# y2w-oc/CMR-Agent

Measured on AMD Instinct MI355X. Metric: registration iters/sec (KITTI 352x1216 img + 16384 pts, 1 geo forward + 10 agent steps), higher is better.
Workload: dtype f32; 1 GPU; BASELINE.json configs[1]: KittiConfig, batch 8 per GPU, 16384 pts, 352x1216 image, 10 agent steps, fp32, hash-filled weights; batch_per_gpu=8, parallelism=batch sharding, no data-path collective

## Files before the change

cmr_agent_amd/models/MultiHeadModel.py:

```python
import itertools
import math

import numpy as np
import torch
import torch.nn as nn

from .. import ops
from ..utils.streams import fork_join
from . import _pack
from ._pack import Planned
from .ImageResNet import ResidualBlock
from .IMGPCEnDecoder import IMGPCEnDecoder
from .PointNN import ConvBNReLURes1D, bcl_from_rows

HEAD_SLOPE = 0.2


class _Head(Planned):

    def __init__(self, config, pc_out, img_out, pc_name, img_name, pc_mid, img_mid):
        super().__init__()
        self.config = config
        f = config.embed_dim
        self.point_fuse_convs = nn.ModuleList([ConvBNReLURes1D(2 * f, f)] +
                                              [ConvBNReLURes1D(f, f) for _ in range(config.pt_head_res_num - 1)])
        setattr(self, pc_name, nn.Sequential(nn.Conv1d(f, pc_mid, kernel_size=1, stride=1, padding=0),
                                             nn.LeakyReLU(HEAD_SLOPE, inplace=True),
                                             nn.Conv1d(pc_mid, pc_out, kernel_size=1, stride=1, padding=0)))
        self.img_res_convs = nn.ModuleList([ResidualBlock(f, f) for _ in range(config.img_fuse_res_num)])
        setattr(self, img_name, nn.Sequential(nn.Conv2d(f, img_mid, 1, 1, 0), nn.LeakyReLU(HEAD_SLOPE, inplace=True),
                                              nn.Conv2d(img_mid, img_out, 1, 1, 0)))
        self._pc_name, self._img_name = pc_name, img_name
        self._pc_out, self._img_out = pc_out, img_out

    def _build_plan(self):
        pc, im = getattr(self, self._pc_name), getattr(self, self._img_name)
        return dict(pc0=_pack.lin(pc[0]), pc2=_pack.lin(pc[2]), im0=_pack.lin(im[0]), im2=_pack.lin(im[2]))

    def points_cl(self, cl):
        self._require_eval()
        p = self.plan()
        x = self.point_fuse_convs[0].rows(cl["pt_feat"], x2=cl["fused_node_feat"], idx2=cl["geo"].gidx)
        for layer in list(self.point_fuse_convs)[1:]:
            x = layer.rows(x)
        pts = ops.linear(ops.linear(x, *p["pc0"], act=ops.ACT_LRELU, act_param=HEAD_SLOPE), *p["pc2"])
        return pts[:, :self._pc_out]

    def pixels_cl(self, cl):
        self._require_eval()
        p = self.plan()
        y = cl["fused_img_feat"]
        for layer in self.img_res_convs:
            y = layer.forward_cl(y)
        B, h, w, f = y.shape
        pix = ops.linear(ops.linear(y.view(B * h * w, f), *p["im0"], act=ops.ACT_LRELU, act_param=HEAD_SLOPE), *p["im2"])
        return pix[:, :self._img_out]

    def trunk_cl(self, cl):
        return fork_join(lambda: self.points_cl(cl), lambda: self.pixels_cl(cl), tag="trunk")


class OverlapDetectionHead(_Head):
    def __init__(self, config):
        super().__init__(config, 2, 2, "pc_overlap_head", "img_overlap_head", 32, 32)

    def finish_cl(self, cl, pts, pix):
        cl["pc_overlap_logits"], cl["img_overlap_logits"] = pts, pix
        return cl

    def forward_cl(self, cl):
        return self.finish_cl(cl, *self.trunk_cl(cl))


MATCH_INLIER_THRES = 3.0
SUBPIXEL_INLIER_THRES = 0.5


def point_xy_float_all(K, pc_in_cam_space):
    K = K.float()
    pc_ = torch.matmul(K if K.dim() == 3 else K.unsqueeze(0), pc_in_cam_space.float())
    return (pc_[:, 0:2, :] / pc_[:, 2:3, :]).contiguous()


def _gt_xy(data_batch, dev):
    xy = data_batch.get('point_xy_float_all')
    if xy is None:
        xy = point_xy_float_all(data_batch['K'].to(dev), data_batch['pc_in_cam_space'].to(dev))
    return xy.to(dev, torch.float32).contiguous()


def _geo_rows(data_batch):
    cl = data_batch.get('_cmr')
    if cl is not None and 'pc_geo_feat' in cl and 'img_geo_feat' in cl:
        return cl['pc_geo_feat'].contiguous(), cl['img_geo_feat'].contiguous()
    pcb, imb = data_batch['pc_geo_feat'], data_batch['img_geo_feat']
    return pcb.permute(0, 2, 1).reshape(-1, pcb.shape[1]).contiguous(), imb.permute(0, 2, 3, 1).contiguous()


def match_features(data_batch, mask, img_overlap=None, want_dist=False):
    pc, img = _geo_rows(data_batch)
    B, h, w, _ = img.shape
    N = pc.shape[0] // B
    dev = pc.device
    xy = _gt_xy(data_batch, dev)
    idx, dist, counts = ops.feat_match(pc, img, mask.to(dev).contiguous(), gt_xy=xy, thr=MATCH_INLIER_THRES, img_overlap=img_overlap,
                                       want_dist=want_dist)
    return idx.view(B, N), dist, counts, w


def match_features_filtered(data_batch, mask, mutual=True, ratio=0.0, excl_radius=2, max_dist=0.0):
    pc, img = _geo_rows(data_batch)
    B, h, w, _ = img.shape
    N = pc.shape[0] // B
    dev = pc.device
    idx, keep, counts, _, _, _ = ops.feat_match_filter(pc, img, mask.to(dev).contiguous(), mutual=mutual, ratio=ratio,
                                                       excl_radius=excl_radius, max_dist=max_dist, gt_xy=_gt_xy(data_batch, dev),
                                                       thr=MATCH_INLIER_THRES)
    return idx.view(B, N), keep.view(B, N), counts, w


def match_features_conf(data_batch, mask, temperature=0.1, min_conf=0.0):
    pc, img = _geo_rows(data_batch)
    B, h, w, _ = img.shape
    N = pc.shape[0] // B
    dev = pc.device
    idx, conf, keep, counts, _, _, _ = ops.match_conf(pc, img, mask.to(dev).contiguous(), temperature=temperature, min_conf=min_conf,
                                                      gt_xy=_gt_xy(data_batch, dev), thr=MATCH_INLIER_THRES)
    return idx.view(B, N), conf.view(B, N), keep.view(B, N), counts, w


def _ratio(counts, num, den):
    c = counts.float()
    return c[:, num] / c[:, den]


class GeometricDistanceHead(_Head):
    def __init__(self, config):
        f = config.embed_dim
        super().__init__(config, f, f, "pc_geo_head", "img_geo_head", f, f)
        self.dist_thres, self.pos_margin, self.neg_margin, self.lambda_geo = 1, 0.1, 1.4, 1

    def finish_cl(self, cl, pts, pix):
        cl["pc_geo_feat"] = ops.l2norm64(pts)
        cl["img_geo_feat"] = ops.l2norm64(pix).view(cl["B"], cl["h"], cl["w"], -1)
        return cl

    def forward_cl(self, cl):
        return self.finish_cl(cl, *self.trunk_cl(cl))

    def cal_match_accuracy(self, data_batch):
        with torch.no_grad():
            _, _, counts, _ = match_features(data_batch, data_batch['pc_mask'])
            ir = _ratio(counts, 1, 0)
            data_batch['matching_ir_per_sample'] = ir
            data_batch['matching_ir'] = ir[0]


_EYE4 = {}


def _eye4(dev):
    key = str(dev)
    if key not in _EYE4:
        _EYE4[key] = torch.eye(4, device=dev).unsqueeze(0)
    return _EYE4[key]


SEARCH_LEVELS = ((4, 1.0, 0.1, 3), (2, 0.5, 0.05, 3), (1, 0.25, 0.025, 3), (0, 0.1, 0.01, 6), (0, 0.03, 0.003, 6))


def pose_search_offsets():
    return np.array(sorted(itertools.product((-1, 0, 1), repeat=6), key=lambda o: (sum(abs(x) for x in o), o)), np.int64)


def pose_search_table(rot_step_deg, trans_step):
    o = pose_search_offsets().astype(np.float64)
    wv = math.radians(float(rot_step_deg)) * o[:, :3]
    th = np.linalg.norm(wv, axis=1)
    W = np.zeros((len(o), 3, 3))
    W[:, 0, 1], W[:, 0, 2], W[:, 1, 2] = -wv[:, 2], wv[:, 1], -wv[:, 0]
    W[:, 1, 0], W[:, 2, 0], W[:, 2, 1] = wv[:, 2], -wv[:, 1], wv[:, 0]
    small = th < 1e-8
    ths = np.where(small, 1.0, th)
    a = np.where(small, 1.0 - th * th / 6.0, np.sin(ths) / ths)
    c = np.where(small, 0.5 - th * th / 24.0, (1.0 - np.cos(ths)) / (ths * ths))
    D = np.tile(np.eye(4), (len(o), 1, 1))
    D[:, :3, :3] += a[:, None, None] * W + c[:, None, None] * (W @ W)
    D[:, :3, 3] = float(trans_step) * o[:, 3:]
    return torch.from_numpy(D)


def _first_min(score):
    P = score.shape[1]
    ar = torch.arange(P, device=score.device)
    k = torch.where(score == score.min(1, keepdim=True).values, ar, torch.full_like(ar, P)).min(1).values
    return torch.where(k < P, k, torch.zeros_like(k))

# ... 434 lines not shown
```

cmr_agent_amd/models/PointNN.py:

```python
import torch
import torch.nn as nn

from .. import ops
from . import _pack
from ._pack import Planned


def rows_from_bcl(x, cpad=None):
    B, C, L = x.shape
    xp = x.permute(0, 2, 1)
    if cpad is None and xp.is_contiguous():
        return xp.reshape(B * L, C)
    if cpad is not None:
        return ops.planar_to_rows(x.contiguous(), cpad)
    return ops.transpose(x.contiguous()).view(B * L, C)


def bcl_from_rows(r, B):
    return r.view(B, -1, r.shape[1]).permute(0, 2, 1)


class MiniPointNet(Planned):
    SLOPE = 0.2

    def __init__(self, in_channels=3, out_channels=64):
        super().__init__()
        self.in_channels = in_channels
        mk = lambda ci: nn.Sequential(nn.Conv1d(ci, out_channels, kernel_size=1, stride=1, padding=0),
                                      nn.BatchNorm1d(out_channels), nn.LeakyReLU(self.SLOPE, inplace=True))
        self.layer_1, self.layer_2, self.layer_3 = mk(in_channels), mk(out_channels), mk(out_channels)

    def _build_plan(self):
        return [_pack.lin(l[0], l[1]) for l in (self.layer_1, self.layer_2, self.layer_3)]

    def rows(self, x1, x2=None, idx2=None, div2=1):
        self._require_eval()
        p = self.plan()
        y = ops.linear(x1, *p[0], x2=x2, idx2=idx2, div2=div2, act=ops.ACT_LRELU, act_param=self.SLOPE)
        y = ops.linear(y, *p[1], act=ops.ACT_LRELU, act_param=self.SLOPE)
        return ops.linear(y, *p[2], act=ops.ACT_LRELU, act_param=self.SLOPE)

    def forward(self, x):
        B = x.shape[0]
        r = rows_from_bcl(x, 4 if self.in_channels < 4 else None)
        return bcl_from_rows(self.rows(r), B)


class ConvBNReLURes1D(Planned):
    SLOPE = 0.2

    def __init__(self, in_channels=3, out_channels=3):
        super().__init__()
        self.in_channels, self.out_channels = in_channels, out_channels
        self.net = nn.Sequential(nn.Conv1d(in_channels, in_channels, kernel_size=1, stride=1, padding=0),
                                 nn.BatchNorm1d(in_channels), nn.LeakyReLU(self.SLOPE, inplace=True),
                                 nn.Conv1d(in_channels, out_channels, kernel_size=1, stride=1, padding=0),
                                 nn.BatchNorm1d(out_channels))
        self.final_relu = nn.LeakyReLU(self.SLOPE, inplace=True)
        if in_channels == out_channels:
            self.shortcut = nn.Identity()
        else:
            self.shortcut = nn.Sequential(nn.Conv1d(in_channels, out_channels, kernel_size=1, stride=1, padding=0),
                                          nn.BatchNorm1d(out_channels))

    def _build_plan(self):
        w1, b1 = _pack.lin(self.net[0], self.net[1])
        w1, b1 = _pack.pad_rows(w1, b1)
        w2, b2 = _pack.lin(self.net[3], self.net[4])
        sc = None if isinstance(self.shortcut, nn.Identity) else _pack.lin(self.shortcut[0], self.shortcut[1])
        b2f = b2 if sc is None else (b2 + sc[1]).contiguous()
        return dict(l1=(w1, b1), l2=(w2, b2), sc=sc, b2f=b2f)

    def rows(self, x1, x2=None, idx2=None, div2=1, res_rows=None):
        self._require_eval()
        p = self.plan()
        fused = ops.cbr_block(x1, p["l1"][0], p["l1"][1], p["l2"][0], p["b2f"], None if p["sc"] is None else p["sc"][0],
                              self.SLOPE, x2=x2, idx2=idx2, div2=div2)
        if fused is not None:
            return fused[0]
        hid = ops.linear(x1, *p["l1"], x2=x2, idx2=idx2, div2=div2, act=ops.ACT_LRELU, act_param=self.SLOPE)
        if p["sc"] is not None:
            res = ops.linear(x1, *p["sc"], x2=x2, idx2=idx2, div2=div2)
        elif x2 is None:
            res = x1
        else:
            res = res_rows if res_rows is not None else ops.concat_rows(x1, x2, idx2, div2)
        return ops.linear(hid, *p["l2"], res=res, act=ops.ACT_LRELU, act_param=self.SLOPE)

    def forward(self, x):
        B = x.shape[0]
        r = rows_from_bcl(x, 8 if self.in_channels == 5 else (4 if self.in_channels < 4 else None))
        return bcl_from_rows(self.rows(r), B)


FUSED_FRONT = True


def _vector_attention(p, q, k, v, rel, rows, nseg, iq, divq, ik, order, offsets, fixed_len):
    pos = ops.linear(ops.linear(rel, *p["d0"], act=ops.ACT_RELU), *p["d2"])
    t, vp = ops.vecattn_prep(q, k, v, pos, rows, iq=iq, divq=divq, ik=ik)
    a = ops.linear(ops.linear(t, *p["g0"], act=ops.ACT_RELU), *p["g2"])
    return ops.segment_softmax(a, vp, nseg, 0.125, order=order, offsets=offsets, fixed_len=fixed_len)


class GroupPointTransformer(Planned):
    def __init__(self, d_points=3, d_model=128):
        super().__init__()
        if d_model != 64:
            raise NotImplementedError("vector-attention kernels are instantiated for d_model = 64")
        c1 = lambda ci, co, bias=True: nn.Conv1d(ci, co, kernel_size=1, stride=1, padding=0, bias=bias)
        self.fc1_0, self.fc1_1, self.fc2 = c1(d_points, d_model), c1(d_points, d_model), c1(d_model, d_points)
        self.fc_delta = nn.Sequential(c1(3, d_model), nn.ReLU(inplace=True), c1(d_model, d_model))
        self.fc_gamma = nn.Sequential(c1(d_model, d_model), nn.ReLU(inplace=True), c1(d_model, d_model))
        self.w_qs, self.w_ks, self.w_vs = c1(d_model, d_model, False), c1(d_model, d_model, False), c1(d_model, d_model, False)
        self.d_model = d_model

    def _build_plan(self):
        wk, _ = _pack.lin(self.w_ks)
        wv, _ = _pack.lin(self.w_vs)
        return dict(fc1_0=_pack.lin(self.fc1_0), fc1_1=_pack.lin(self.fc1_1), fc2=_pack.lin(self.fc2),
                    d0=_pack.lin(self.fc_delta[0]), d2=_pack.lin(self.fc_delta[2]), g0=_pack.lin(self.fc_gamma[0]),
                    g2=_pack.lin(self.fc_gamma[2]), wq=_pack.lin(self.w_qs)[0], wkv=torch.cat([wk, wv], 0).contiguous())

    def rows(self, xyz4, feat, node4, node_feat, gidx, offsets, order):
        self._require_eval()
        p = self.plan()
        R, S = feat.shape[0], node_feat.shape[0]
        q = ops.linear(ops.linear(node_feat, *p["fc1_1"]), p["wq"])
        if FUSED_FRONT and p["d0"][0].shape == (64, 4):
            a, vp = ops.vecattn_front(q, xyz4, node4, gidx, p["d0"], p["d2"], p["g0"], p["g2"], R, iq=gidx, feat=feat,
                                      fc1=p["fc1_0"], wkv=p["wkv"])
            res = ops.segment_softmax(a, vp, S, 0.125, order=order, offsets=offsets, fixed_len=0)
        else:
            kv = ops.linear(ops.linear(feat, *p["fc1_0"]), p["wkv"])
            rel = ops.rel_pos(xyz4, node4, R, ib=gidx)
            res = _vector_attention(p, q, kv[:, 0:64], kv[:, 64:128], rel, R, S, gidx, 1, None, order, offsets, 0)
        return ops.linear(res, *p["fc2"], res=node_feat)

    def forward(self, xyz, xyz_features, node, node_features, idx):
        B, N, M = xyz.shape[0], xyz.shape[2], node.shape[2]
        gidx = ops.index_to_global(idx.contiguous(), M)
        offsets, order = ops.csr_build(gidx, B, N, M)
        out = self.rows(rows_from_bcl(xyz, 4), rows_from_bcl(xyz_features), rows_from_bcl(node, 4),
                        rows_from_bcl(node_features), gidx, offsets, order)
        return bcl_from_rows(out, B)


class KnnPointTransformer(Planned):
    def __init__(self, d_points=3, d_model=128, k=16):
        super().__init__()
        if d_model != 64 or k != 16:
            raise NotImplementedError("kNN transformer kernels are instantiated for d_model = 64, k = 16")
        self.fc1, self.fc2 = nn.Linear(d_points, d_model), nn.Linear(d_model, d_points)
        self.fc_delta = nn.Sequential(nn.Linear(3, d_model), nn.ReLU(inplace=True), nn.Linear(d_model, d_model))
        self.fc_gamma = nn.Sequential(nn.Linear(d_model, d_model), nn.ReLU(inplace=True), nn.Linear(d_model, d_model))
        self.w_qs = nn.Linear(d_model, d_model, bias=False)
        self.w_ks = nn.Linear(d_model, d_model, bias=False)
        self.w_vs = nn.Linear(d_model, d_model, bias=False)
        self.k = k

    def _build_plan(self):
        wq, wk, wv = (_pack.lin(l)[0] for l in (self.w_qs, self.w_ks, self.w_vs))
        return dict(fc1=_pack.lin(self.fc1), fc2=_pack.lin(self.fc2), d0=_pack.lin(self.fc_delta[0]),
                    d2=_pack.lin(self.fc_delta[2]), g0=_pack.lin(self.fc_gamma[0]), g2=_pack.lin(self.fc_gamma[2]),
                    wqkv=torch.cat([wq, wk, wv], 0).contiguous())

    def rows(self, node4, feat, knn):
        self._require_eval()
        p = self.plan()
        S = feat.shape[0]
        qkv = ops.linear(ops.linear(feat, *p["fc1"]), p["wqkv"])
        if FUSED_FRONT and p["d0"][0].shape == (64, 4):
            a, vp = ops.vecattn_front(qkv[:, 0:64], node4, node4, knn, p["d0"], p["d2"], p["g0"], p["g2"], S * 16, divq=16,
                                      diva=16, kv=qkv[:, 64:192], ik=knn)
            res = ops.segment_softmax(a, vp, S, 0.125, fixed_len=16)
        else:
            rel = ops.rel_pos(node4, node4, S * 16, diva=16, ib=knn)
            res = _vector_attention(p, qkv[:, 0:64], qkv[:, 64:128], qkv[:, 128:192], rel, S * 16, S, None, 16, knn, None,
                                    None, 16)
        return ops.linear(res, *p["fc2"], res=feat)

    def forward(self, xyz, features):
        B, M = xyz.shape[0], xyz.shape[2]
        node4 = rows_from_bcl(xyz, 4)
        knn = ops.knn16(node4, B, M).view(-1)
        return bcl_from_rows(self.rows(node4, rows_from_bcl(features), knn), B)
```

cmr_agent_amd/ops.py:

```python
import math
import os

import torch

from . import _lib

ACT_NONE, ACT_RELU, ACT_LRELU, ACT_GELU, ACT_ELU1 = 0, 1, 2, 3, 4
f32 = torch.float32
GRID_Y_MAX = 65535


def _stream():
    return torch.cuda.current_stream().cuda_stream


def _p(t):
    return None if t is None else t.data_ptr()


def _rows(t, name="tensor"):
    if t.dim() != 2 or t.stride(1) != 1 or t.dtype != f32 or not t.is_cuda:
        raise ValueError("%s must be a 2-D float32 device tensor with unit inner stride, got %s %s %s" % (
            name, tuple(t.shape), t.stride(), t.dtype))
    return t
# ... 44 lines not shown
        k2 = x2.shape[1]
    if kw != k1 + k2 or w.stride(1) != 1 or w.stride(0) < kw:
        raise ValueError("weight shape %s / strides %s do not match k1+k2=%d" % (tuple(w.shape), w.stride(), k1 + k2))
    ldw = w.stride(0) if n_out > 1 else kw
    if out is None:
        out = torch.empty((rows, n_out), dtype=f32, device=x1.device)
    _rows(out, "out")
    if res is not None:
        _rows(res, "res")
    if _AB_SKIP_LINEAR:
        key = (rows, n_out, x1.device)
        if key not in _AB_ZERO:
            _AB_ZERO[key] = torch.zeros((rows, n_out), dtype=f32, device=x1.device)
        return _AB_ZERO[key]
    if CONV_BF16 and LINEAR_BF16 and x2 is None and ldw == kw and rows >= LINEAR_BF16_MIN_ROWS and k1 in (32, 64, 128) and n_out <= 128 and n_out % 4 == 0:
        rc = _lib.call("cmr_linear_rows_bf16_f32", _p(x1), _ld(x1), k1, _p(w), kw, _p(bias), _p(res), _ld(res) if res is not None else 0,
                       int(res_mod), _p(out), _ld(out), rows, n_out, act, float(act_param), _stream(), allow_unsupported=True)
        if rc != _lib.UNSUPPORTED:
            return out
    _lib.call("cmr_linear_f32", _p(x1), _ld(x1), k1, _p(x2), _ld(x2) if x2 is not None else 0, k2, _p(_i32(idx2)),
              int(div2), _p(w), ldw, _p(bias), _p(res), _ld(res) if res is not None else 0, int(res_mod), _p(out),
              _ld(out), rows, n_out, act, float(act_param), _stream())
    return out


def cbr_block(x1, w1, b1, w2, b2, wsc, slope, x2=None, idx2=None, div2=1, rows_per_batch=None, want_y=True,
              want_colmax=False):
    _rows(x1, "x1")
    rows, k1 = x1.shape
    kx = k1 + (x2.shape[1] if x2 is not None else 0)
    ch, co = w1.shape[0], w2.shape[0]
    if w1.shape[1] != kx or w2.shape[1] != ch or (wsc is not None and tuple(wsc.shape) != (co, kx)):
        raise ValueError("cbr_block: inconsistent weight shapes")
    rpb = rows if rows_per_batch is None else rows_per_batch
    B = rows // rpb
    if want_colmax and (rpb % 32 or rows % rpb):
        return None
    y = torch.empty((rows, co), dtype=f32, device=x1.device) if want_y else None
    ntiles = (rows + 31) // 32
    part = torch.empty((ntiles, co), dtype=f32, device=x1.device) if want_colmax else None
    s1 = b1.stride(0) if b1.dim() == 2 else 0
    s2 = b2.stride(0) if b2.dim() == 2 else 0
    rc = _lib.call("cmr_cbr_block_bf16_f32" if CONV_BF16 else "cmr_cbr_block_f32", _p(x1), _ld(x1), k1, _p(x2), _ld(x2) if x2 is not None else 0, _p(_i32(idx2)),
                   int(div2), kx, ch, co, _p(w1), _p(b1), s1, _p(w2), _p(b2), s2, _p(wsc), _p(y), co, _p(part), rows, rpb,
                   float(slope), _stream(), allow_unsupported=True)
    if rc == _lib.UNSUPPORTED:
        return None
    cm = None
    if want_colmax == "partials":
        return y, part
    if want_colmax:
        cm = colmax_partials(part, B, rpb // 32)
    return y, cm


def colmax_partials(part, B, tiles_per_batch):
    co = part.shape[1]
    cm = torch.empty((B, co), dtype=f32, device=part.device)
    _lib.call("cmr_colmax_partials_f32", _p(part), _p(cm), B, int(tiles_per_batch), co, _stream())
    return cm


COLMAX_BIAS2 = os.environ.get("CMR_COLMAX_BIAS2", "fp32")


def colmax_bias2(part, B, tiles_per_batch, w1, b1, w2, b2, want_g=False):
    C = part.shape[1]
    n1, n2 = w1.shape[0], w2.shape[0]
    if COLMAX_BIAS2 == "0" or (COLMAX_BIAS2 == "fp32" and CONV_BF16) or C != 64 or n1 % 4 or n2 % 4 or not (w1.is_contiguous() and w2.is_contiguous()) or w1.shape[1] != C or w2.shape[1] != C:
        return None
    y1 = torch.empty((B, n1), dtype=f32, device=part.device)
    y2 = torch.empty((B, n2), dtype=f32, device=part.device)
    g = torch.empty((B, C), dtype=f32, device=part.device) if want_g else None
    rc = _lib.call("cmr_colmax_bias2_f32", _p(part), B, int(tiles_per_batch), C, _p(w1), _p(b1), n1, _p(w2), _p(b2), n2, _p(g), _p(y1), _p(y2), _stream(),
                   allow_unsupported=True)
    return None if rc == _lib.UNSUPPORTED else (y1, y2, g)


def layernorm64(x, gamma, beta, eps, res=None, out=None):
    _rows(x, "x")
    if out is None:
        out = torch.empty((x.shape[0], 64), dtype=f32, device=x.device)
    _lib.call("cmr_layernorm64_f32", _p(x), _ld(x), _p(gamma), _p(beta), float(eps), _p(res),
              _ld(res) if res is not None else 0, _p(out), _ld(out), x.shape[0], _stream())
    return out


CONV_BF16 = False
BF16_CHAINS = True
BF16_STORE = True
STRIDE2_FRAGS = True
WINOGRAD = True
WINO_MIN_TILES = 64


TOWER_CU_BUDGET = 160
TOWER_CU_BUDGET_F32 = 0


TOWER_SLICES_F32 = int(os.environ.get("CMR_TOWER_SLICES", "1"))


import threading

_policy = threading.local()

# ... 2035 lines not shown
```

cmr_agent_amd/utils/workmodel.py:

```python
import torch

from .. import _lib

FP32_MFMA_PEAK = 157.3e12
HBM_PEAK = 8.0e12
RIDGE = FP32_MFMA_PEAK / HBM_PEAK
F = 4


def _linear(a):
    rows, k1, n = a["rows"], a["k1"], a["n_out"]
    k2 = a["k2"] if a["x2"] else 0
    src2 = 0
    if a["x2"]:
        src2 = rows * k2 if a["idx2"] else max(rows // max(a["div2"], 1), 1) * k2
    by = F * (rows * k1 + src2 + rows * n + n * (k1 + k2) + (rows * n if a["res"] and not a["res_mod"] else 0))
    return 2.0 * rows * (k1 + k2) * n, by


def _cbr(a):
    rows, kx, ch, co, k1 = a["rows"], a["kx"], a["ch"], a["co"], a["k1"]
    w = kx * ch + ch * co + (kx * co if a["wsc"] else 0)
    src2 = 0
    if a["x2"]:
        src2 = rows * (kx - k1) if a["idx2"] else max(rows // max(a["div2"], 1), 1) * (kx - k1)
    return 2.0 * rows * w, F * (rows * k1 + src2 + (rows * co if a["y"] else 0) + w)


def _conv(a, stride=None):
    s = a.get("stride", 1) if stride is None else stride
    B, H, W, ci, co, pool = a["B"], a["H"], a["W"], a["Cin"], a["Cout"], a.get("pool", 1)
    opix = B * ((H - 1) // s + 1) * ((W - 1) // s + 1)
    by = F * (B * H * W * ci + opix * co / (pool * pool) + (opix * co if a["res"] else 0) + 9 * ci * co)
    return 2.0 * 9 * ci * co * opix, by


def _conv_io(a):
    s = a.get("stride", 1)
    B, H, W, ci, co, pool = a["B"], a["H"], a["W"], a["Cin"], a["Cout"], a.get("pool", 1)
    opix = B * ((H - 1) // s + 1) * ((W - 1) // s + 1)
    by = ((2 if a["x_bf16"] else F) * B * H * W * ci + (2 if a["y_bf16"] else F) * opix * co / (pool * pool)
          + (2 if a.get("res_bf16") else F) * (opix * co if a["res"] else 0) + F * 9 * ci * co)
    return 2.0 * 9 * ci * co * opix, by


def _heads(a):
    w = 2 * 128 * 128 + sum(256 * a[p + "_n0"] + a[p + "_n0"] * a[p + "_n1"] + a[p + "_n1"] * a[p + "_n2"] for p in "rtv")
    return 2.0 * a["B"] * w, F * (a["B"] * a["npix"] * 128 + w)


def _vecattn(a):
    rows = a["rows"]
    if a["feat"]:
        return rows * 2.0 * (3 * 4096 + 192 + 4096 + 2 * 4096), rows * (256 + 256 + 32 + 512)
    return rows * 2.0 * (192 + 4096 + 2 * 4096), rows * (512 + 256 + 32 + 512)


WORK = {
    "cmr_linear_f32": _linear,
    "cmr_cbr_block_f32": _cbr,
    "cmr_cbr_block_bf16_f32": _cbr,
    "cmr_colmax_partials_f32": lambda a: (0, F * a["B"] * a["tiles_per_batch"] * a["C"]),
    "cmr_colmax_bias2_f32": lambda a: (2.0 * a["B"] * a["C"] * (a["n1"] + a["n2"]),
                                       F * (a["B"] * a["tiles_per_batch"] * a["C"] + (a["C"] + 1 + a["B"]) * (a["n1"] + a["n2"]))),
    "cmr_layernorm64_f32": lambda a: (0, F * a["rows"] * 64 * (3 if a["res"] else 2)),
    "cmr_conv3x3_nhwc_f32": _conv,
    "cmr_conv3x3_wino_nhwc_f32": lambda a: _conv(a, 1),
    "cmr_conv3x3_wino_stats_nhwc_f32": lambda a: (2.0 * 9 * a["Cin"] * a["Cout"] * a["B"] * a["H"] * a["W"],
                                                  F * (a["B"] * a["H"] * a["W"] * (a["Cin"] + a["Cout"]) + 9 * a["Cin"] * a["Cout"])),
    "cmr_bn_stats_from_sums_f32": lambda a: (0, F * a["parts"] * 2 * a["C"]),
    "cmr_conv3x3_wino_bnbwd_nhwc_f32": lambda a: (2.0 * 9 * a["Cin"] * a["Cout"] * a["B"] * a["H"] * a["W"],
                                                  F * (a["B"] * a["H"] * a["W"] * (a["Cin"] + 2 * a["Cout"]) + 9 * a["Cin"] * a["Cout"])),
    "cmr_bn_bwd_from_sums_f32": lambda a: (0, F * a["rows"] * a["C"] * 3),
    "cmr_conv3x3_s2_nhwc_f32": lambda a: _conv(a, 2),
    "cmr_conv3x3_bf16_nhwc_f32": _conv,
    "cmr_conv3x3_bf16io_nhwc": _conv_io,
    "cmr_conv3x3_bf16_pro_nhwc_f32": lambda a: (2.0 * 9 * a["Cin"] * a["Cout"] * a["B"] * a["H"] * a["W"],
                                                F * (a["B"] * a["H"] * a["W"] * (a["Cin"] + a["Cout"]) + 9 * a["Cin"] * a["Cout"])),
    "cmr_stem_block_f32": lambda a: (2.0 * (81 + 1728 + 192) * a["B"] * a["H"] * a["W"], a["B"] * a["H"] * a["W"] * (F * 3 + (2 if a.get("out_bf16") else F) * 64)),
    "cmr_avgpool_nhwc_f32": lambda a: (0, F * a["B"] * a["H"] * a["W"] * a["C"] * (1 + 1.0 / (a["kh"] * a["kw"]))),
    "cmr_upsample_concat_f32": lambda a: (0, F * a["B"] * a["H"] * a["W"] * (2 * a["C1"] + a["C2"] * (1 + 1.0 / a["scale"] ** 2))),
    "cmr_patchify_nhwc_f32": lambda a: (0, 2 * F * a["B"] * a["H"] * a["W"] * a["C"]),
    "cmr_transpose_f32": lambda a: (0, 2 * F * a["batch"] * a["R"] * a["Cn"]),
    "cmr_linear_rows_bf16_f32": lambda a: (2.0 * a["rows"] * a["k"] * a["n_out"], F * (a["rows"] * (a["k"] + a["n_out"] * (2 if a["res"] else 1)) + a["k"] * a["n_out"])),
    "cmr_patch_embed_f32": lambda a: (2.0 * a["B"] * (a["H"] // a["P"]) * (a["W"] // a["P"]) * a["P"] * a["P"] * a["C"] * a["n_out"],
                                     F * (a["B"] * a["H"] * a["W"] * a["C"] + a["B"] * (a["H"] // a["P"]) * (a["W"] // a["P"]) * a["n_out"] + a["P"] * a["P"] * a["C"] * a["n_out"])),
    "cmr_mha_f32": lambda a: (4.0 * a["B"] * a["Tq"] * a["Tk"] * 64, F * 64 * a["B"] * (2 * a["Tq"] + 2 * a["Tk"])),
    "cmr_mha_expf_f32": lambda a: (4.0 * a["B"] * a["Tq"] * a["Tk"] * 64, F * 64 * a["B"] * (2 * a["Tq"] + 2 * a["Tk"])),
    "cmr_mha_ln_f32": lambda a: (4.0 * a["B"] * a["Tq"] * a["Tk"] * 64 + 2.0 * 64 * a["B"] * (64 * a["Tq"] + 128 * a["Tk"]),
                                F * 64 * a["B"] * (2 * a["Tq"] + a["Tk"])),
    "cmr_la_reduce_f32": lambda a: (2.0 * a["B"] * a["S"] * 576, F * a["B"] * a["S"] * 128),
    "cmr_la_apply_f32": lambda a: (2.0 * a["B"] * a["L"] * 576, F * a["B"] * a["L"] * 128),
    "cmr_agent_heads_f32": _heads,
    "cmr_agent_heads_train_f32": _heads,
    "cmr_ln64_linear_f32": lambda a: (2.0 * 64 * (a["rows_x"] * a["n_out_x"] + (a["rows_y"] * a["n_out_y"] if a["y"] else 0)),
                                      F * (a["rows_x"] * (64 + a["n_out_x"]) + (a["rows_y"] * (64 + a["n_out_y"]) if a["y"] else 0)
                                           + 64 * (a["n_out_x"] + (a["n_out_y"] if a["y"] else 0)))),
    "cmr_ln64_linear_bf16_f32": lambda a: (2.0 * 64 * (a["rows_x"] * a["n_out_x"] + (a["rows_y"] * a["n_out_y"] if a["y"] else 0)),
                                      F * (a["rows_x"] * (64 + a["n_out_x"]) + (a["rows_y"] * (64 + a["n_out_y"]) if a["y"] else 0)
                                           + 64 * (a["n_out_x"] + (a["n_out_y"] if a["y"] else 0)))),
    "cmr_vit_out_ffn_f32": lambda a: (2.0 * a["rows"] * (4096 + 2 * 65536), F * (a["rows"] * 192 + 4096 + 2 * 65536)),
    "cmr_vit_out_ffn16_f32": lambda a: (2.0 * a["rows"] * (4096 + 2 * 65536), F * (a["rows"] * 192 + 4096 + 2 * 65536)),
    "cmr_vit_out_ffn_bf16_f32": lambda a: (2.0 * a["rows"] * (4096 + 2 * 65536), F * (a["rows"] * 192 + 4096 + 2 * 65536)),
    "cmr_la_kv_state_f32": lambda a: (2.0 * a["B"] * a["S"] * (2 * 4096 + 576), F * (a["B"] * a["S"] * 64 + 2 * 4096)),
    "cmr_la_kv_state_bf16_f32": lambda a: (2.0 * a["B"] * a["S"] * (2 * 4096 + 576), F * (a["B"] * a["S"] * 64 + 2 * 4096)),
    "cmr_la_query_layer_f32": lambda a: (2.0 * a["B"] * a["L"] * (4096 + 576 + 4096 + 16384 + 8192),
                                         F * (a["B"] * a["L"] * 128 + 2 * 4096 + 16384 + 8192)),
    "cmr_la_query_layer_bf16_f32": lambda a: (2.0 * a["B"] * a["L"] * (4096 + 576 + 4096 + 16384 + 8192),
                                         F * (a["B"] * a["L"] * 128 + 2 * 4096 + 16384 + 8192)),
    "cmr_vecattn_front_f32": _vecattn,
    "cmr_focal_metrics_f32": lambda a: (0, a["rows"] * 16),
    "cmr_circle_loss_f32": lambda a: (2.0 * a["B"] * a["n"] * a["n"] * 64, F * a["B"] * a["n"] * 128),
    "cmr_planar_to_rows_f32": lambda a: (0, F * a["B"] * a["N"] * (a["C"] + a["Cpad"])),
# ... 189 lines not shown
```

include/cmr_hip.h:

```cpp
#ifndef CMR_HIP_H
#define CMR_HIP_H
#include <stdint.h>

#ifdef __cplusplus
extern "C" {
#endif

typedef struct ihipStream_t* hipStream_t;

#define CMR_OK 0
#define CMR_EINVAL -1
#define CMR_ELAUNCH -2
#define CMR_EUNSUPPORTED -3

enum { CMR_ACT_NONE = 0, CMR_ACT_RELU = 1, CMR_ACT_LRELU = 2, CMR_ACT_GELU = 3, CMR_ACT_ELU1 = 4 };


int cmr_linear_f32(const float* x1, int64_t ld1, int k1, const float* x2, int64_t ld2, int k2, const int32_t* idx2,
                   int64_t div2, const float* w, int64_t ldw, const float* bias, const float* res, int64_t ldres,
                   int64_t res_mod, float* y, int64_t ldy, int64_t rows, int n_out, int act, float act_param,
                   hipStream_t stream);
int cmr_cbr_block_f32(const float* x1, int64_t ld1, int k1, const float* x2, int64_t ld2, const int32_t* idx2,
                      int64_t div2, int kx, int ch, int co, const float* w1, const float* b1, int64_t b1_stride,
                      const float* w2, const float* b2, int64_t b2_stride, const float* wsc, float* y, int64_t ldy,
                      float* colmax_part, int64_t rows, int64_t rows_per_batch, float slope, hipStream_t stream);
int cmr_cbr_block_bf16_f32(const float* x1, int64_t ld1, int k1, const float* x2, int64_t ld2, const int32_t* idx2,
                           int64_t div2, int kx, int ch, int co, const float* w1, const float* b1, int64_t b1_stride,
                           const float* w2, const float* b2, int64_t b2_stride, const float* wsc, float* y, int64_t ldy,
                           float* colmax_part, int64_t rows, int64_t rows_per_batch, float slope, hipStream_t stream);
int cmr_colmax_partials_f32(const float* part, float* out, int B, int tiles_per_batch, int C, hipStream_t stream);
int cmr_colmax_bias2_f32(const float* part, int B, int tiles_per_batch, int C, const float* w1, const float* b1, int n1, const float* w2,
                         const float* b2, int n2, float* g, float* y1, float* y2, hipStream_t stream);

int cmr_layernorm64_f32(const float* x, int64_t ldx, const float* gamma, const float* beta, float eps, const float* res,
                        int64_t ldres, float* y, int64_t ldy, int64_t rows, hipStream_t stream);

int cmr_conv3x3_nhwc_f32(const float* x, int B, int H, int W, int Cin, const float* w, const float* bias,
                         const float* res, const float* post, float* y, int Cout, int stride, float slope, int pool,
                         hipStream_t stream);

int cmr_conv3x3_wino_nhwc_f32(const float* x, int B, int H, int W, int Cin, const float* u, const float* bias,
                              const float* res, const float* post, float* y, int Cout, float slope, int pool,
                              int cu_budget, int slices, hipStream_t stream);
int64_t cmr_conv3x3_wino_stats_parts(int B, int H, int W, int Cin, int Cout, int cu_budget, int slices);
int cmr_conv3x3_wino_stats_nhwc_f32(const float* x, int B, int H, int W, int Cin, const float* u, const float* bias, float* y, int Cout,
                                    int cu_budget, int slices, float* part, int64_t parts, hipStream_t stream);
int cmr_conv3x3_wino_bnbwd_nhwc_f32(const float* dy, int B, int H, int W, int Cin, const float* u, float* dx, int Cout, const float* bn_x,
                                    const float* bn_stat, float bn_slope, int cu_budget, int slices, float* part, int64_t parts,
                                    hipStream_t stream);
int cmr_conv3x3_s2_nhwc_f32(const float* x, int B, int H, int W, int Cin, const float* wfrag, const float* bias, const float* res,
                            const float* post, float* y, int Cout, float slope, hipStream_t stream);
int cmr_stem_block_f32(const float* x_nchw, const float* w_a, const float* b_a, const float* w3, const float* w1,
                       const float* b_b, float* tmp_nchw, void* y_nhwc, int out_bf16, int B, int H, int W, float slope,
                       hipStream_t stream);

int cmr_avgpool_nhwc_f32(const float* x, float* y, int B, int H, int W, int C, int kh, int kw, hipStream_t stream);

int cmr_upsample_concat_f32(const float* f, const float* proxy, float* out, int B, int H, int W, int C1, int C2,
                            int scale, hipStream_t stream);

int cmr_patchify_nhwc_f32(const float* x, float* out, int B, int H, int W, int C, int P, hipStream_t stream);
int cmr_patch_embed_f32(const float* x_nhwc, int B, int H, int W, int C, int P, const float* w, int64_t ldw, const float* bias,
                        const float* res, int64_t ldres, int64_t res_mod, float* y, int64_t ldy, int n_out, hipStream_t stream);
int cmr_linear_rows_bf16_f32(const float* x, int64_t ldx, int k, const float* w, int64_t ldw, const float* bias, const float* res,
                             int64_t ldres, int64_t res_mod, float* y, int64_t ldy, int64_t rows, int n_out, int act, float act_param,
                             hipStream_t stream);

int cmr_transpose_f32(const float* x, float* y, int batch, int R, int Cn, hipStream_t stream);


int cmr_mha_f32(const float* q, int64_t ldq, const float* k, int64_t ldk, const float* v, int64_t ldv, float* o,
                int64_t ldo, int B, int Tq, int Tk, hipStream_t stream);
int cmr_mha_expf_f32(const float* q, int64_t ldq, const float* k, int64_t ldk, const float* v, int64_t ldv, float* o, int64_t ldo, int B,
                     int Tq, int Tk, hipStream_t stream);
int cmr_mha_ln_f32(const float* x, int64_t ldx, const float* y, int64_t ldy, const float* gamma, const float* beta, float eps,
                   const float* wq_frag, const float* wkv_frag, const float* bq, const float* bk, const float* bv, float* o, int64_t ldo,
                   int B, int Tq, int Tk, hipStream_t stream);
int64_t cmr_la_reduce_workspace_bytes(int B, int S);
int cmr_la_reduce_f32(const float* kf, int64_t ldk, const float* v, int64_t ldv, float* kvsum, void* workspace,
                      int64_t workspace_bytes, int B, int S, hipStream_t stream);
int cmr_la_apply_f32(const float* qf, int64_t ldq, const float* kvsum, float* msg, int64_t ldm, int B, int L, int S,
                     float eps, hipStream_t stream);

// ... 449 lines not shown
```

Baseline: 418.4 registration iters/s.

## Fuse chains of row-wise linear layers into one LDS-resident MFMA kernel

```diff
diff --git a/cmr_agent_amd/csrc/row_chain.hip b/cmr_agent_amd/csrc/row_chain.hip
--- /dev/null
+++ b/cmr_agent_amd/csrc/row_chain.hip
@@ -0,0 +1,244 @@
+#include "cmr_common.h"
+
+namespace {
+
+__device__ __attribute__((aligned(16))) float rc_zero[16] = {0.f};
+
+struct RcArgs {
+  const float* x1; int64_t ld1;
+  const float* x2; int64_t ld2; const int32_t* idx2; int64_t div2;
+  int k1;
+  const float* w1; const float* b1;
+  const float* w2; const float* b2;
+  const float* w3; const float* b3;
+  float s1, s2, s3;
+  float* y; int64_t ldy;
+  int64_t rows;
+};
+
+template <int C, int K, int KP>
+__device__ __forceinline__ void rc_stage(float* Ws, float* Bs, const float* __restrict__ w, const float* __restrict__ b, int tid) {
+  constexpr int P = 32 * ((C + 31) / 32), LD = KP + 4;
+  for (int e = tid; e < P * (KP / 4); e += 512) {
+    const int n = e / (KP / 4), c = (e % (KP / 4)) * 4;
+    const bool ok = n < C && c < K;
+    *reinterpret_cast<f32x4*>(&Ws[n * LD + c]) = *reinterpret_cast<const f32x4*>(ok ? w + (int64_t)n * K + c : rc_zero);
+  }
+  for (int e = tid; e < P; e += 512) Bs[e] = (b && e < C) ? b[e] : 0.f;
+}
+
+template <int G, int T, int LD>
+__device__ __forceinline__ void rc_gemm(const float* wl, const f32x4 (&in)[G], f32x16 (&acc)[T]) {
+#pragma unroll
+  for (int t = 0; t < T; ++t)
+#pragma unroll
+    for (int r = 0; r < 16; ++r) acc[t][r] = 0.f;
+  f32x4 wc[T], wn[T];
+#pragma unroll
+  for (int t = 0; t < T; ++t) wc[t] = *reinterpret_cast<const f32x4*>(wl + t * 32 * LD);
+#pragma unroll
+  for (int g = 0; g < G; ++g) {
+    if (g + 1 < G) {
+#pragma unroll
+      for (int t = 0; t < T; ++t) wn[t] = *reinterpret_cast<const f32x4*>(wl + t * 32 * LD + (g + 1) * 8);
+    }
+#pragma unroll
+    for (int j = 0; j < 4; ++j)
+#pragma unroll
+      for (int t = 0; t < T; ++t) acc[t] = cmr_mfma32(wc[t][j], in[g][j], acc[t]);
+    __builtin_amdgcn_sched_barrier(0);
+#pragma unroll
+    for (int t = 0; t < T; ++t) wc[t] = wn[t];
+  }
+}
+
+template <int T>
+__device__ __forceinline__ void rc_act(const f32x16 (&acc)[T], const float* bl, float slope, f32x4 (&out)[4 * T]) {
+#pragma unroll
+  for (int t = 0; t < T; ++t)
+#pragma unroll
+    for (int q = 0; q < 4; ++q) {
+      const f32x4 bv = *reinterpret_cast<const f32x4*>(bl + t * 32 + q * 8);
+#pragma unroll
+      for (int e = 0; e < 4; ++e) {
+        const float v = acc[t][4 * q + e] + bv[e];
+        out[4 * t + q][e] = v > 0.f ? v : v * slope;
+      }
+    }
+}
+
+template <int G, int TL, int TC, int LD, int CL, bool NORM>
+__device__ __forceinline__ void rc_last(const float* wl, const float* bl, const f32x4 (&in)[G], float slope, float* yrow, bool valid, int h) {
+  static_assert(!NORM || (CL == 64 && TL == 2 && TC == 2), "l2norm epilogue: 64 channels");
+#pragma unroll
+  for (int c0 = 0; c0 < TL; c0 += TC) {
+    f32x16 acc[TC];
+    rc_gemm<G, TC, LD>(wl + c0 * 32 * LD, in, acc);
+    f32x4 ov[4 * TC];
+    rc_act<TC>(acc, bl + c0 * 32, slope, ov);
+    if constexpr (NORM) {
+      float s[8];
+#pragma unroll
+      for (int i = 0; i < 8; ++i) {
+        const float p = fmaf(ov[i][0], ov[i][0], ov[i][1] * ov[i][1]) + fmaf(ov[i][2], ov[i][2], ov[i][3] * ov[i][3]);
+        s[i] = p + cmr_xhalf(p);
+      }
+      const float qq = ((s[0] + s[1]) + (s[2] + s[3])) + ((s[4] + s[5]) + (s[6] + s[7]));
+      const float d = fmaxf(sqrtf(qq), 1e-12f);
+#pragma unroll
+      for (int i = 0; i < 8; ++i)
+#pragma unroll
+        for (int e = 0; e < 4; ++e) ov[i][e] = ov[i][e] / d;
+    }
+#pragma unroll
+    for (int i = 0; i < 4 * TC; ++i) cmr_pin(ov[i]);
+    if (valid) {
+#pragma unroll
+      for (int t = 0; t < TC; ++t)
+#pragma unroll
+        for (int q = 0; q < 4; ++q) {
+          const int c = (c0 + t) * 32 + q * 8;
+          if (c + 8 <= CL) *reinterpret_cast<f32x4*>(yrow + c) = ov[4 * t + q];
+          else if (c + 4 <= CL && h == 0) *reinterpret_cast<f32x4*>(yrow + c) = ov[4 * t + q];
+        }
+    }
+  }
+}
+
+template <int K0, int C1, int C2, int C3, bool NORM>
+__global__ __launch_bounds__(512) void row_chain_kernel(const RcArgs a) {
+  constexpr int KP = K0 < 8 ? 8 : K0, GX = KP / 8;
+  constexpr bool THREE = C3 > 0;
+  constexpr int T1 = (C1 + 31) / 32, T2 = (C2 + 31) / 32, T3 = (C3 + 31) / 32;
+  constexpr int LD1 = KP + 4, LD2 = C1 + 4, LD3 = C2 + 4;
+  constexpr int CL = THREE ? C3 : C2, TL = THREE ? T3 : T2, TC = TL >= 2 ? 2 : 1;
+  static_assert(C1 % 32 == 0 && (!THREE || C2 % 32 == 0) && CL % 4 == 0 && TL % TC == 0 && K0 % 4 == 0, "served widths");
+  extern __shared__ __attribute__((aligned(16))) float smem[];
+  float* W1s = smem;
+  float* W2s = W1s + 32 * T1 * LD1;
+  float* W3s = W2s + 32 * T2 * LD2;
+  float* B1s = W3s + 32 * T3 * LD3;
+  float* B2s = B1s + 32 * T1;
+  float* B3s = B2s + 32 * T2;
+  const int tid = threadIdx.x, lane = tid & 63;
+  const int wave = __builtin_amdgcn_readfirstlane(tid >> 6);
+  const int h = lane >> 5, l31 = lane & 31;
+  const uint32_t rows = (uint32_t)a.rows;
+  rc_stage<C1, K0, KP>(W1s, B1s, a.w1, a.b1, tid);
+  rc_stage<C2, C1, C1>(W2s, B2s, a.w2, a.b2, tid);
+  if constexpr (THREE) rc_stage<C3, C2, C2>(W3s, B3s, a.w3, a.b3, tid);
+  __syncthreads();
+
+  const uint32_t ntiles = (rows + 31) / 32, tstride = gridDim.x * 8;
+  const float* x2b = a.x2 ? a.x2 : a.x1;
+  const int32_t* izero = reinterpret_cast<const int32_t*>(rc_zero);
+  auto load_idx = [&](uint32_t tile) -> int32_t {
+    const uint32_t row = tile * 32 + l31;
+    const uint32_t ok = (a.idx2 != nullptr && tile < ntiles && row < rows) ? 1u : 0u;
+    return (a.idx2 ? a.idx2 : izero)[ok * row];
+  };
+  auto load_x = [&](uint32_t tile, int32_t idxv, f32x4 (&xf)[GX]) {
+    uint32_t row = tile * 32 + l31;
+    row = (tile < ntiles && row < rows) ? row : 0;
+    if constexpr (K0 == 4) {
+      const f32x4 v = *reinterpret_cast<const f32x4*>(a.x1 + (int64_t)row * a.ld1);
+#pragma unroll
+      for (int e = 0; e < 4; ++e) xf[0][e] = h ? 0.f : v[e];
+    } else {
+      const int64_t r2 = a.idx2 ? (int64_t)idxv : (int64_t)(row / (uint32_t)a.div2);
+      const float* p1 = a.x1 + (int64_t)row * a.ld1 + 4 * h;
+      const float* p2 = x2b + r2 * a.ld2 + 4 * h - a.k1;
+#pragma unroll
+      for (int g = 0; g < GX; ++g) xf[g] = *reinterpret_cast<const f32x4*>((g * 8 + 4 * h < a.k1 ? p1 : p2) + g * 8);
+    }
+  };
+
+  uint32_t tile = blockIdx.x * 8 + wave;
+  f32x4 xf[GX], xn[GX];
+  int32_t idn = load_idx(tile);
+  load_x(tile, idn, xf);
+  idn = load_idx(tile + tstride);
+  for (; tile < ntiles; tile += tstride) {
+    const uint32_t row = tile * 32 + l31;
+    const bool valid = row < rows;
+    load_x(tile + tstride, idn, xn);
+    idn = load_idx(tile + 2 * tstride);
+    float* yrow = a.y + (int64_t)(valid ? row : 0) * a.ldy + 4 * h;
+    f32x16 acc1[T1];
+    rc_gemm<GX, T1, LD1>(W1s + l31 * LD1 + 4 * h, xf, acc1);
+    f32x4 h1[4 * T1];
+    rc_act<T1>(acc1, B1s + 4 * h, a.s1, h1);
+    if constexpr (THREE) {
+      f32x16 acc2[T2];
+      rc_gemm<4 * T1, T2, LD2>(W2s + l31 * LD2 + 4 * h, h1, acc2);
+      f32x4 h2[4 * T2];
+      rc_act<T2>(acc2, B2s + 4 * h, a.s2, h2);
+      rc_last<4 * T2, TL, TC, LD3, CL, NORM>(W3s + l31 * LD3 + 4 * h, B3s + 4 * h, h2, a.s3, yrow, valid, h);
+    } else {
+      rc_last<4 * T1, TL, TC, LD2, CL, NORM>(W2s + l31 * LD2 + 4 * h, B2s + 4 * h, h1, a.s2, yrow, valid, h);
+    }
+#pragma unroll
+    for (int g = 0; g < GX; ++g) xf[g] = xn[g];
+  }
+}
+
+constexpr int rc_pad32(int c) { return 32 * ((c + 31) / 32); }
+constexpr size_t rc_smem_bytes(int k0, int c1, int c2, int c3) {
+  const int kp = k0 < 8 ? 8 : k0;
+  return (size_t)(rc_pad32(c1) * (kp + 4) + rc_pad32(c2) * (c1 + 4) + rc_pad32(c3) * (c2 + 4) + rc_pad32(c1) + rc_pad32(c2) + rc_pad32(c3)) *
+         sizeof(float);
+}
+
+constexpr int RC_SHAPES[][4] = {{4, 64, 64, 64}, {128, 64, 64, 64}, {64, 64, 64, 0}, {64, 32, 4, 0}, {64, 64, 192, 0}};
+int rc_shape(int k0, int c1, int c2, int c3, int l2norm) {
+  for (int i = 0; i < (int)(sizeof(RC_SHAPES) / sizeof(RC_SHAPES[0])); ++i)
+    if (RC_SHAPES[i][0] == k0 && RC_SHAPES[i][1] == c1 && RC_SHAPES[i][2] == c2 && RC_SHAPES[i][3] == c3) return (l2norm && i != 2) ? -1 : i;
+  return -1;
+}
+
+int64_t rc_grid(size_t smem, int64_t rows, int max_workgroups) {
+  const int64_t ntiles = (rows + 31) / 32;
+  const int64_t cap = max_workgroups > 0 ? max_workgroups : 256 * (smem > 80 * 1024 ? 1 : 2);
+  const int64_t grid = (ntiles + 7) / 8;
+  return grid > cap ? cap : grid;
+}
+
+template <int K0, int C1, int C2, int C3, bool NORM>
+int launch_rc(const RcArgs& a, int max_workgroups, hipStream_t stream) {
+  constexpr size_t smem = rc_smem_bytes(K0, C1, C2, C3);
+  static_assert(smem <= 160 * 1024, "weights must fit in LDS");
+  static CmrSmemCache granted{};
+  if (cmr_grant_smem(reinterpret_cast<const void*>(row_chain_kernel<K0, C1, C2, C3, NORM>), smem, granted) != CMR_OK) return CMR_ELAUNCH;
+  const int64_t grid = rc_grid(smem, a.rows, max_workgroups);
+  hipLaunchKernelGGL((row_chain_kernel<K0, C1, C2, C3, NORM>), dim3((unsigned)grid), dim3(512), smem, stream, a);
+  return cmr_launch_status();
+}
+
+}
+
+extern "C" int cmr_row_chain_grid(int k0, int c1, int c2, int c3, int l2norm, int64_t rows, int max_workgroups) {
+  CMR_REQUIRE(rows > 0);
+  if (rc_shape(k0, c1, c2, c3, l2norm) < 0 || rows >= (int64_t)0x7fffffc0) return CMR_EUNSUPPORTED;
+  return (int)rc_grid(rc_smem_bytes(k0, c1, c2, c3), rows, max_workgroups);
+}
+
+extern "C" int cmr_row_chain_f32(const float* x1, int64_t ld1, int k1, const float* x2, int64_t ld2, const int32_t* idx2, int64_t div2,
+                                 int k0, int c1, int c2, int c3, const float* w1, const float* b1, float slope1, const float* w2,
+                                 const float* b2, float slope2, const float* w3, const float* b3, float slope3, int l2norm, float* y,
+                                 int64_t ldy, int64_t rows, int max_workgroups, hipStream_t stream) {
+  CMR_REQUIRE(x1 && w1 && w2 && y && rows > 0 && k0 > 0 && c1 > 0 && c2 > 0 && c3 >= 0 && (c3 == 0) == (w3 == nullptr));
+  CMR_REQUIRE(k1 > 0 && k1 % 4 == 0 && k1 <= k0 && (k1 == k0 || x2) && ld1 % 4 == 0 && ld1 >= k1 && cmr_aligned16(x1));
+  if (x2) CMR_REQUIRE(k0 >= 8 && ld2 % 4 == 0 && ld2 >= k0 - k1&& cmr_aligned16(x2) && (idx2 || div2 >= 1));
+  const int cl = c3 ? c3 : c2;
+  CMR_REQUIRE(ldy % 4 == 0 && ldy >= cl && cmr_aligned16(y) && cmr_aligned16(w1) && cmr_aligned16(w2) && (!w3 || cmr_aligned16(w3)));
+  const int shape = rc_shape(k0, c1, c2, c3, l2norm);
+  if (shape < 0 || rows >= (int64_t)0x7fffffc0) return CMR_EUNSUPPORTED;
+  const RcArgs a{x1, ld1, x2, ld2, idx2, div2 < 1 ? 1 : div2, k1, w1, b1, w2, b2, w3, b3, slope1, slope2, slope3, y, ldy, rows};
+  switch (shape) {
+    case 0: return launch_rc<4, 64, 64, 64, false>(a, max_workgroups, stream);
+    case 1: return launch_rc<128, 64, 64, 64, false>(a, max_workgroups, stream);
+    case 2: return l2norm ? launch_rc<64, 64, 64, 0, true>(a, max_workgroups, stream) : launch_rc<64, 64, 64, 0, false>(a, max_workgroups, stream);
+    case 3: return launch_rc<64, 32, 4, 0, false>(a, max_workgroups, stream);
+    default: return launch_rc<64, 64, 192, 0, false>(a, max_workgroups, stream);
+  }
+}
diff --git a/cmr_agent_amd/models/MultiHeadModel.py b/cmr_agent_amd/models/MultiHeadModel.py
--- a/cmr_agent_amd/models/MultiHeadModel.py
+++ b/cmr_agent_amd/models/MultiHeadModel.py
@@ -31,6 +31,7 @@
         setattr(self, img_name, nn.Sequential(nn.Conv2d(f, img_mid, 1, 1, 0), nn.LeakyReLU(HEAD_SLOPE, inplace=True),
                                               nn.Conv2d(img_mid, img_out, 1, 1, 0)))
         self._pc_name, self._img_name = pc_name, img_name
+        self._l2norm = False
         self._pc_out, self._img_out = pc_out, img_out
 
     def _build_plan(self):
@@ -43,8 +44,15 @@
         x = self.point_fuse_convs[0].rows(cl["pt_feat"], x2=cl["fused_node_feat"], idx2=cl["geo"].gidx)
         for layer in list(self.point_fuse_convs)[1:]:
             x = layer.rows(x)
-        pts = ops.linear(ops.linear(x, *p["pc0"], act=ops.ACT_LRELU, act_param=HEAD_SLOPE), *p["pc2"])
-        return pts[:, :self._pc_out]
+        return self._head_rows(x, p["pc0"], p["pc2"])[:, :self._pc_out]
+
+    def _head_rows(self, x, l0, l2):
+        y = ops.row_chain(x, [l0 + (ops.ACT_LRELU, HEAD_SLOPE), l2 + (ops.ACT_NONE, 0.0)], l2norm=self._l2norm, min_rows=ops.ROW_CHAIN_MIN_ROWS)
+        if y is None:
+            y = ops.linear(ops.linear(x, *l0, act=ops.ACT_LRELU, act_param=HEAD_SLOPE), *l2)
+            if self._l2norm:
+                y = ops.l2norm64(y)
+        return y
 
     def pixels_cl(self, cl):
         self._require_eval()
@@ -53,8 +61,7 @@
         for layer in self.img_res_convs:
             y = layer.forward_cl(y)
         B, h, w, f = y.shape
-        pix = ops.linear(ops.linear(y.view(B * h * w, f), *p["im0"], act=ops.ACT_LRELU, act_param=HEAD_SLOPE), *p["im2"])
-        return pix[:, :self._img_out]
+        return self._head_rows(y.view(B * h * w, f), p["im0"], p["im2"])[:, :self._img_out]
 
     def trunk_cl(self, cl):
         return fork_join(lambda: self.points_cl(cl), lambda: self.pixels_cl(cl), tag="trunk")
@@ -139,10 +146,11 @@
         f = config.embed_dim
         super().__init__(config, f, f, "pc_geo_head", "img_geo_head", f, f)
         self.dist_thres, self.pos_margin, self.neg_margin, self.lambda_geo = 1, 0.1, 1.4, 1
+        self._l2norm = True
 
     def finish_cl(self, cl, pts, pix):
-        cl["pc_geo_feat"] = ops.l2norm64(pts)
-        cl["img_geo_feat"] = ops.l2norm64(pix).view(cl["B"], cl["h"], cl["w"], -1)
+        cl["pc_geo_feat"] = pts
+        cl["img_geo_feat"] = pix.view(cl["B"], cl["h"], cl["w"], -1)
         return cl
 
     def forward_cl(self, cl):
diff --git a/cmr_agent_amd/models/PointNN.py b/cmr_agent_amd/models/PointNN.py
--- a/cmr_agent_amd/models/PointNN.py
+++ b/cmr_agent_amd/models/PointNN.py
@@ -36,6 +36,10 @@
     def rows(self, x1, x2=None, idx2=None, div2=1):
         self._require_eval()
         p = self.plan()
+        fused = ops.row_chain(x1, [(w, b, ops.ACT_LRELU, self.SLOPE) for w, b in p], x2=x2, idx2=idx2, div2=div2,
+                              min_rows=ops.ROW_CHAIN_MIN_ROWS)
+        if fused is not None:
+            return fused
         y = ops.linear(x1, *p[0], x2=x2, idx2=idx2, div2=div2, act=ops.ACT_LRELU, act_param=self.SLOPE)
         y = ops.linear(y, *p[1], act=ops.ACT_LRELU, act_param=self.SLOPE)
         return ops.linear(y, *p[2], act=ops.ACT_LRELU, act_param=self.SLOPE)
@@ -126,7 +130,9 @@
         self._require_eval()
         p = self.plan()
         R, S = feat.shape[0], node_feat.shape[0]
-        q = ops.linear(ops.linear(node_feat, *p["fc1_1"]), p["wq"])
+        q = ops.row_chain(node_feat, [p["fc1_1"] + (ops.ACT_NONE, 0.0), (p["wq"], None, ops.ACT_NONE, 0.0)], min_rows=ops.ROW_CHAIN_MIN_ROWS)
+        if q is None:
+            q = ops.linear(ops.linear(node_feat, *p["fc1_1"]), p["wq"])
         if FUSED_FRONT and p["d0"][0].shape == (64, 4):
             a, vp = ops.vecattn_front(q, xyz4, node4, gidx, p["d0"], p["d2"], p["g0"], p["g2"], R, iq=gidx, feat=feat,
                                       fc1=p["fc1_0"], wkv=p["wkv"])
@@ -169,7 +175,9 @@
         self._require_eval()
         p = self.plan()
         S = feat.shape[0]
-        qkv = ops.linear(ops.linear(feat, *p["fc1"]), p["wqkv"])
+        qkv = ops.row_chain(feat, [p["fc1"] + (ops.ACT_NONE, 0.0), (p["wqkv"], None, ops.ACT_NONE, 0.0)], min_rows=ops.ROW_CHAIN_MIN_ROWS)
+        if qkv is None:
+            qkv = ops.linear(ops.linear(feat, *p["fc1"]), p["wqkv"])
         if FUSED_FRONT and p["d0"][0].shape == (64, 4):
             a, vp = ops.vecattn_front(qkv[:, 0:64], node4, node4, knn, p["d0"], p["d2"], p["g0"], p["g2"], S * 16, divq=16,
                                       diva=16, kv=qkv[:, 64:192], ik=knn)
diff --git a/cmr_agent_amd/ops.py b/cmr_agent_amd/ops.py
--- a/cmr_agent_amd/ops.py
+++ b/cmr_agent_amd/ops.py
@@ -120,6 +120,55 @@
     if want_colmax:
         cm = colmax_partials(part, B, rpb // 32)
     return y, cm
+
+
+ROW_CHAIN = os.environ.get("CMR_ROW_CHAIN", "1") != "0"
+ROW_CHAIN_MIN_ROWS = 17
+
+
+def _chain_slope(act, act_param):
+    if act == ACT_NONE:
+        return 1.0
+    if act == ACT_RELU:
+        return 0.0
+    return float(act_param) if act == ACT_LRELU else None
+
+
+def _chain_dims(x1, layers, x2):
+    k0 = x1.shape[1] + (x2.shape[1] if x2 is not None else 0)
+    dims = [k0] + [l[0].shape[0] for l in layers]
+    return dims + [0] * (4 - len(dims))
+
+
+def row_chain_grid(x1, layers, x2=None, l2norm=False, max_grid=0, rows=None):
+    k0, c1, c2, c3 = _chain_dims(x1, layers, x2)
+    g = _lib.load().cmr_row_chain_grid(k0, c1, c2, c3, int(bool(l2norm)), int(x1.shape[0] if rows is None else rows), int(max_grid))
+    return None if g < 0 else g
+
+
+def row_chain(x1, layers, x2=None, idx2=None, div2=1, l2norm=False, max_grid=0, min_rows=0):
+    _rows(x1, "x1")
+    rows = x1.shape[0]
+    if not ROW_CHAIN or _AB_SKIP_LINEAR or rows < max(min_rows, 1) or len(layers) not in (2, 3):
+        return None
+    if CONV_BF16 and LINEAR_BF16 and rows >= LINEAR_BF16_MIN_ROWS:
+        return None
+    if x2 is not None:
+        _rows(x2, "x2")
+    slopes = [_chain_slope(l[2], l[3]) for l in layers]
+    k = x1.shape[1] + (x2.shape[1] if x2 is not None else 0)
+    for (w, b, _, _), s in zip(layers, slopes):
+        if s is None or w.dim() != 2 or w.shape[1] != k or not w.is_contiguous() or (b is not None and not b.is_contiguous()):
+            return None
+        k = w.shape[0]
+    k0, c1, c2, c3 = _chain_dims(x1, layers, x2)
+    y = torch.empty((rows, k), dtype=f32, device=x1.device)
+    l3 = layers[2] if len(layers) == 3 else (None, None)
+    rc = _lib.call("cmr_row_chain_f32", _p(x1), _ld(x1), x1.shape[1], _p(x2), _ld(x2) if x2 is not None else 0, _p(_i32(idx2)), int(div2),
+                   k0, c1, c2, c3, _p(layers[0][0]), _p(layers[0][1]), slopes[0], _p(layers[1][0]), _p(layers[1][1]), slopes[1],
+                   _p(l3[0]), _p(l3[1]), slopes[2] if len(layers) == 3 else 1.0, int(bool(l2norm)), _p(y), k, rows, int(max_grid), _stream(),
+                   allow_unsupported=True)
+    return None if rc == _lib.UNSUPPORTED else y
 
 
 def colmax_partials(part, B, tiles_per_batch):
diff --git a/cmr_agent_amd/utils/workmodel.py b/cmr_agent_amd/utils/workmodel.py
--- a/cmr_agent_amd/utils/workmodel.py
+++ b/cmr_agent_amd/utils/workmodel.py
@@ -27,6 +27,15 @@
     return 2.0 * rows * w, F * (rows * k1 + src2 + (rows * co if a["y"] else 0) + w)
 
 
+def _row_chain(a):
+    rows, k0, k1 = a["rows"], a["k0"], a["k1"]
+    w = k0 * a["c1"] + a["c1"] * a["c2"] + a["c2"] * a["c3"]
+    src2 = 0
+    if a["x2"]:
+        src2 = rows * (k0 - k1) if a["idx2"] else max(rows // max(a["div2"], 1), 1) * (k0 - k1)
+    return 2.0 * rows * w, F * (rows * k1 + src2 + rows * (a["c3"] or a["c2"]) + w)
+
+
 def _conv(a, stride=None):
     s = a.get("stride", 1) if stride is None else stride
     B, H, W, ci, co, pool = a["B"], a["H"], a["W"], a["Cin"], a["Cout"], a.get("pool", 1)
@@ -59,6 +68,7 @@
 WORK = {
     "cmr_linear_f32": _linear,
     "cmr_cbr_block_f32": _cbr,
+    "cmr_row_chain_f32": _row_chain,
     "cmr_cbr_block_bf16_f32": _cbr,
     "cmr_colmax_partials_f32": lambda a: (0, F * a["B"] * a["tiles_per_batch"] * a["C"]),
     "cmr_colmax_bias2_f32": lambda a: (2.0 * a["B"] * a["C"] * (a["n1"] + a["n2"]),
diff --git a/include/cmr_hip.h b/include/cmr_hip.h
--- a/include/cmr_hip.h
+++ b/include/cmr_hip.h
@@ -29,6 +29,11 @@
                            const float* w2, const float* b2, int64_t b2_stride, const float* wsc, float* y, int64_t ldy,
                            float* colmax_part, int64_t rows, int64_t rows_per_batch, float slope, hipStream_t stream);
 int cmr_colmax_partials_f32(const float* part, float* out, int B, int tiles_per_batch, int C, hipStream_t stream);
+int cmr_row_chain_f32(const float* x1, int64_t ld1, int k1, const float* x2, int64_t ld2, const int32_t* idx2, int64_t div2, int k0,
+                      int c1, int c2, int c3, const float* w1, const float* b1, float slope1, const float* w2, const float* b2,
+                      float slope2, const float* w3, const float* b3, float slope3, int l2norm, float* y, int64_t ldy, int64_t rows,
+                      int max_workgroups, hipStream_t stream);
+int cmr_row_chain_grid(int k0, int c1, int c2, int c3, int l2norm, int64_t rows, int max_workgroups);
 int cmr_colmax_bias2_f32(const float* part, int B, int tiles_per_batch, int C, const float* w1, const float* b1, int n1, const float* w2,
                          const float* b2, int n2, float* g, float* y1, float* y2, hipStream_t stream);
 
```

After: 420.5 registration iters/s (median of 6 runs). Within noise of the previous version (+0.5%).
